# BenjSta/bernoulli-var-speech-codec

Measured on AMD Instinct MI355X. Metric: audio-seconds coded per wall-second (encode+decode), 22.05 kHz @ 3 kbit/s, higher is better.
Workload: dtype f32; 1 GPU; BASELINE configs[1]: batch 64 x 5 s utterances per GPU, config_varBitRate @ 3000 bit/s (35 bits/frame), full encode -> BigVGAN decode; one batch at a time on one stream; frames_per_utterance=430, weights=seeded synthetic (checkpoints are LFS pointers), gather=none, streams=1

## Files before the change

bernoulli-var-speech-codec_amd/csrc/bvc_internal.h:

```cpp
#pragma once
#include <hip/hip_runtime.h>
#include <stdint.h>
#include <string>
#include <vector>

#include "../../include/bvcodec.h"

namespace bvc {

void set_error(const char *fmt, ...);

#define BVC_HIP_TRY(expr)                                                              \
    do {                                                                               \
        hipError_t e_ = (expr);                                                        \
        if (e_ != hipSuccess) {                                                        \
            bvc::set_error("%s failed: %s (%s:%d)", #expr, hipGetErrorString(e_), __FILE__, __LINE__); \
            return BVC_EHIP;                                                           \
        }                                                                              \
    } while (0)

enum ProbeKind { PK_NONE = 0, PK_LINEAR = 1, PK_GRU = 2, PK_CONV = 3, PK_BATCHED = 4, PK_STFT = 5, PK_POST = 6 };
struct ProbeScope {
    hipStream_t s; int slot;
    ProbeScope(int kind, hipStream_t stream);
// ... 168 lines not shown
    const int   *mel_off;
    const float *mel_w;
    int num_mels;
    int kmax;
};
int launch_stft_logmel(const FrontendTables &t, const float *wav, int B, long long L, long long T,
                       int pad_left, float scale, float *mel, hipStream_t s, const long long *lens = nullptr);
__host__ __device__ inline long long ragged_frames(long long len, long long L, int pad_left) {
    len = len < 0 ? 0 : (len > L ? L : len);
    const long long pr = 1024 - 256 - pad_left;
    if (len <= pad_left || len <= pr) return 0;
    return (len + pad_left + pr - 1024) / 256 + 1;
}
int launch_ragged_bits(float *bits, const float *d_bits, float dflt, const long long *lens, int B, long long L, long long T,
                       int pad_left, hipStream_t s);
int launch_ragged_mask(float *codes, const long long *lens, int B, long long L, long long T, int z, int pad_left, hipStream_t s);

int launch_resample_poly(const float *x, int B, long long Lin, const double *h, int ntaps, int up, int down,
                         long long n_pre_remove, float *y, long long n_out, hipStream_t s);
int launch_peak_normalize(float *x, int B, long long L, hipStream_t s);
int launch_pack_codes(const float *codes, long long frames, int z, int nbits, unsigned char *out, hipStream_t s);
int launch_unpack_codes(const unsigned char *in, long long frames, int z, int nbits, float *codes, hipStream_t s);
int launch_pack_rows(const float *codes, const float *bits, int B, int k, int z, int kstride, unsigned char *out, hipStream_t s);
int launch_unpack_rows(const unsigned char *in, const unsigned char *present, const float *bits, const int *row_off, int B, int k,
                       int z, int kstride, float *codes, hipStream_t s);
int launch_conceal_select(const unsigned char *present, long long kstride, const float *bits, float dflt, const int *row_off, int B,
                          long long k, float *sel, hipStream_t s);

struct ConvLayer {
    int cin;
    int cout;
    int ntiles;
    int ks;
    int dil;
    const float *wp;
    const float *wp4;
    const float *wp2;
    const float *bias;
    const float *act_a;
    const float *act_ib;
    const float *aa_up;
    const float *aa_down;
};
enum ConvEpi { CE_STORE = 0, CE_RES = 1, CE_RES_ACC = 2, CE_RES_ACC_DIV = 3 };
#ifdef BVC_PHASE_PROBE
int phase_probe_read(unsigned long long *out, int reset);
#endif
struct ConvWindow {
    long long in_bs, out_bs, row_begin, t_origin;
    const int *row_age = nullptr;
    int age_rate = 0;
};
int conv_kernels_init();
enum : unsigned { AMPK_C8 = 1u, AMPK_C16 = 2u, AMPK_ALL = 3u };
unsigned amp_kernels_default();
struct AmpLaunch { long long tiles, workgroups; int tile_rows; };
extern AmpLaunch g_last_amp_launch;
int launch_snakebeta_test(const float *x, long long n, float a, float ib, float *y, hipStream_t s);
int launch_conv_mfma(const ConvLayer &c, const float *in, long long Lin, float *out, long long Lout,
                     int B, int epi, const float *res, const float *acc, float divisor, hipStream_t s,
                     const ConvWindow *win = nullptr, const long long *row_lim = nullptr,
                     long long in_bs = 0,
                     int shift = 0);
int launch_amp_pair(const ConvLayer &c1, const ConvLayer &c2, const float *x, long long L, float *out, int B, int epi,
                    const float *acc, float divisor, hipStream_t s, const ConvWindow *win = nullptr, unsigned kernels = AMPK_ALL,
                    bool sym = false,
                    long long bs = 0);
int launch_conv_post(const float *in, long long Lin, int C, int ks, const float *w, const float *bias,
                     const float *act_a, const float *act_ib, float div, float *wav, long long n_out,
                     int B, hipStream_t s, const ConvWindow *win = nullptr, const long long *n_rows = nullptr,
                     const float *aa_up = nullptr, const float *aa_down = nullptr,
                     bool sym = false,
                     long long in_bs = 0);
int launch_ragged_limits(long long *lim, const long long *frames, const long long *lengths, int B, long long T, long long n_max,
                         int n_up, const int *up_rates, hipStream_t s);

}
```

bernoulli-var-speech-codec_amd/csrc/k_vocoder.hip:

```cpp
#include <cstdlib>
#include <type_traits>

#include "bvc_internal.h"

namespace bvc {

typedef float f32x4 __attribute__((ext_vector_type(4)));

__device__ __forceinline__ void divide_if(bool div, f32x4 &v, float d) {
    if (div) {
        asm volatile("" ::: "memory");
#pragma unroll
        for (int e = 0; e < 4; ++e) v[e] = v[e] / d;
    }
}

__device__ __forceinline__ unsigned div_tpb(unsigned bid, unsigned tpb_magic) { return __umulhi(bid, tpb_magic); }
static inline unsigned tpb_magic_of(unsigned d) { return d <= 1u ? 0xFFFFFFFFu : (unsigned)(0x100000000ull / d) + 1u; }

__device__ __forceinline__ __amdgpu_buffer_rsrc_t rows_rsrc(const float *base, long long L, int C) {
    return __builtin_amdgcn_make_buffer_rsrc(const_cast<float *>(base), 0, (int)(L * C * 4), 0x00020000);
}
__device__ __forceinline__ f32x4 rows_load4(__amdgpu_buffer_rsrc_t rs, int row, int C, int c0) {
    return __builtin_bit_cast(f32x4, __builtin_amdgcn_raw_buffer_load_b128(rs, (row * C + c0) * 4, 0, 0));
// ... 190 lines not shown
    const int j0 = run * R, j1 = j0 + R < ndst ? j0 + R : ndst;
    if (j0 >= j1) return;
    const int last = L - 1 > 0x7FFFFFFFll ? 0x7FFFFFFF : (int)(L - 1);
    const int glo = src_first > 0 ? src_first : 0;
    const int ghi = src_first + nsrc - 1 < last ? src_first + nsrc - 1 : last;
    const f32x2 aa = *reinterpret_cast<const f32x2 *>(act_a + c), bb = *reinterpret_cast<const f32x2 *>(act_ib + c);
    float f[12], g[12];
#pragma unroll
    for (int k = 0; k < 12; ++k) { f[k] = fu[k]; g[k] = fd[k]; }
    auto pair = [&](int t, f32x2 &ev, f32x2 &od) {
        const int tc = t < 0 ? 0 : (t > last ? last : t);
        f32x2 xr[7];
#pragma unroll
        for (int k = 0; k < 7; ++k) {
            int q = tc - 3 + k;
            q = q < glo ? glo : (q > ghi ? ghi : q);
            xr[k] = *reinterpret_cast<const f32x2 *>(src + (q - src_first) * S + c);
        }
        f32x2 ue = splat2(f[1]) * xr[5], uo = splat2(f[0]) * xr[6];
#pragma unroll
        for (int k = 1; k < 6; ++k) {
            ue = __builtin_elementwise_fma(splat2(f[2 * k + 1]), xr[5 - k], ue);
            uo = __builtin_elementwise_fma(splat2(f[2 * k]), xr[6 - k], uo);
        }
        ev = snakebeta2(ue * splat2(2.0f), aa, bb);
        od = snakebeta2(uo * splat2(2.0f), aa, bb);
        if (t < 0) od = ev;
        if (t > last) ev = od;
    };
    f32x2 pe[6], po[6];
    const int tfirst = dst_first + j0;
#pragma unroll
    for (int k = 0; k < 6; ++k) pair(tfirst - 3 + k, pe[k], po[k]);
#pragma unroll 1
    for (int j = j0; j < j1; ++j) {
        const int t = dst_first + j;
        f32x2 ne, no;
        pair(t + 3, ne, no);
        f32x2 y = splat2(g[0]) * po[0];
#pragma unroll
        for (int k = 1; k < 6; ++k) {
            y = __builtin_elementwise_fma(splat2(g[2 * k - 1]), pe[k], y);
            y = __builtin_elementwise_fma(splat2(g[2 * k]), po[k], y);
        }
        y = __builtin_elementwise_fma(splat2(g[11]), ne, y);
        if (t < 0) y = splat2(0.0f);
        *reinterpret_cast<float2 *>(dst + j * S + c) = make_float2(y[0], y[1]);
#pragma unroll
        for (int k = 0; k < 5; ++k) { pe[k] = pe[k + 1]; po[k] = po[k + 1]; }
        pe[5] = ne; po[5] = no;
    }
}

template <int C, int MT, int OCC, bool ALIAS, int CS = 1, bool AA = false, bool SYM = false>
__global__ __launch_bounds__(256, OCC) void amp_pair_kernel(AmpArgs a) {
    static_assert(!(SYM && AA), "a filtered stage is a causal stage");
#ifdef BVC_PHASE_PROBE
    unsigned long long last_ = __builtin_readcyclecounter();
#endif
    extern __shared__ __attribute__((aligned(16))) float lds[];
    constexpr int S = C + 2;
    constexpr int NT = (C + 15) / 16;
    constexpr int C4 = C / 4;
    constexpr int TR = (4 / CS) * MT * 16;
    constexpr int NTL = NT / CS;
    static_assert((CS == 1 || CS == 2 || CS == 4) && NT % CS == 0, "the waves along the columns must divide the column tiles");
    constexpr int CGU = C4 < 16 / NTL ? C4 : 16 / NTL;
    constexpr bool W4 = C >= 32 && CGU % 4 == 0;
    const int tid = threadIdx.x, lane = tid & 63;
    const int wave = __builtin_amdgcn_readfirstlane(tid >> 6);
    const int r = lane & 15, g = lane >> 4;
    const int ks = a.ks, dil = a.dil;
    constexpr int AAH = AA ? 5 : 0;
    const int TT = TR - (ks - 1) - 2 * AAH;
    const unsigned nwg = gridDim.x, per = (nwg + 7u) >> 3;
    unsigned bid = (blockIdx.x & 7u) * per + (blockIdx.x >> 3);
    if (bid >= a.ntile) return;
    const int b = a.tiles_per_batch == 1 ? (int)bid : (int)div_tpb(bid, a.tpb_magic);
    const long long t0 = a.row_begin + (long long)(bid - (unsigned)b * (unsigned)a.tiles_per_batch) * TT;
    const int halo1 = (ks - 1) * dil;
    const int rows1 = TR + halo1;
    float *t1 = lds;
    float *t2 = (ALIAS || AA) ? lds : lds + rows1 * S;
    const float *xb = a.x + (long long)b * a.bs;
    const long long tbase = t0 - (SYM ? (ks - 1) / 2 : ks - 1) - AAH;
    const int rowsA = rows1 > TR + ks - 1 ? rows1 : TR + ks - 1;
    float *traw = lds + rowsA * S;
    (void)traw;

    if constexpr (AA) {
        constexpr int NLD = ((TR + 10 * 5 + 2 * AAH) * C4 + 255) / 256;
        f32x4 v[NLD];
        const int total = (rows1 + 2 * AAH) * C4;
        const __amdgpu_buffer_rsrc_t rs = rows_rsrc(xb, a.L, C);
        const int xfirst = (int)(tbase - halo1) - AAH;
#pragma unroll
        for (int i = 0; i < NLD; ++i) {
            const int idx = tid + i * 256;
            const int row = idx / C4, c4 = idx - row * C4;
            v[i] = rows_load4(rs, xfirst + row, C, c4 * 4);
        }
#pragma unroll
        for (int i = 0; i < NLD; ++i) {
            const int idx = tid + i * 256;
            if (idx < total) {
                const int row = idx / C4, c4 = idx - row * C4;
                float2 *dst = reinterpret_cast<float2 *>(traw + row * S + c4 * 4);
                dst[0] = make_float2(v[i][0], v[i][1]);
                dst[1] = make_float2(v[i][2], v[i][3]);
            }
        }
        __syncthreads();
        aa_rows<C>(traw, xfirst, rows1 + 2 * AAH, a.L, t1, xfirst + AAH, rows1, S, a.a1, a.ib1, a.fu1, a.fd1);
    } else {
        constexpr int NLD = ((TR + 10 * 5) * C4 + 255) / 256;
        f32x4 v[NLD];
        const int total = rows1 * C4;
        const __amdgpu_buffer_rsrc_t rs = rows_rsrc(xb, a.L, C);
        const int tfirst = (int)(tbase - (SYM ? halo1 / 2 : halo1));
#pragma unroll
        for (int i = 0; i < NLD; ++i) {
            const int idx = tid + i * 256;
            const int row = idx / C4, c4 = idx - row * C4;
            v[i] = rows_load4(rs, tfirst + row, C, c4 * 4);
        }
#pragma unroll
        for (int i = 0; i < NLD; ++i) {
            const int idx = tid + i * 256;
            if (idx < total) {
                const int row = idx / C4, c4 = idx - row * C4;
                const f32x4 aa = *reinterpret_cast<const f32x4 *>(a.a1 + c4 * 4);
                const f32x4 bb = *reinterpret_cast<const f32x4 *>(a.ib1 + c4 * 4);
                f32x4 o;
#pragma unroll
                for (int e = 0; e < 4; e += 2) {
                    const f32x2 o2 = snakebeta2((f32x2){v[i][e], v[i][e + 1]}, (f32x2){aa[e], aa[e + 1]}, (f32x2){bb[e], bb[e + 1]});
                    o[e] = o2[0]; o[e + 1] = o2[1];
                }
                float2 *dst = reinterpret_cast<float2 *>(t1 + row * S + c4 * 4);
                dst[0] = make_float2(o[0], o[1]);
                dst[1] = make_float2(o[2], o[3]);
            }
        }
    }
    __syncthreads();
    PHASE(0);

    const int mbase = (wave / CS) * MT * 16;
    const int nt0 = (wave % CS) * NTL;
    f32x4 acc[MT][NTL];
    auto mma = [&](const float *tile, int d, const float *wp) {
#pragma unroll
        for (int i = 0; i < MT; ++i)
#pragma unroll
            for (int n = 0; n < NTL; ++n) acc[i][n] = (f32x4){0.f, 0.f, 0.f, 0.f};
        const float *wl = wp + lane;
        constexpr int CPT = C4 / CGU;
        const int nch = ks * CPT;
        constexpr int G4 = W4 ? CGU / 4 : CGU;
        typedef typename std::conditional<W4, f32x4, float>::type BW;
        BW bcur[G4][NTL], bnxt[G4][NTL];
        auto loadb = [&](BW (&dstb)[G4][NTL], int q) {
            if constexpr (W4) {
                const f32x4 *wq = reinterpret_cast<const f32x4 *>(wp) + (long long)q * G4 * NT * 64 + lane;
#pragma unroll
                for (int u = 0; u < G4; ++u)
#pragma unroll
                    for (int n = 0; n < NTL; ++n) dstb[u][n] = wq[(u * NT + nt0 + n) * 64];
            } else {
                const float *wq = wl + (long long)q * CGU * NT * 64;
#pragma unroll
                for (int u = 0; u < CGU; ++u)
#pragma unroll
                    for (int n = 0; n < NTL; ++n) dstb[u][n] = wq[(u * NT + nt0 + n) * 64];
            }
        };
        auto bfrag = [&](const BW (&bw)[G4][NTL], int u, int n) -> float {
            if constexpr (W4) return bw[u >> 2][n][u & 3];
            else return bw[u][n];
        };
        auto compute = [&](const BW (&bw)[G4][NTL], int q) {
            const int j = q / CPT, cg0 = (q - j * CPT) * CGU;
            const float *arow = tile + (mbase + r + j * d) * S + g;
#pragma unroll
            for (int u = 0; u < CGU; ++u) {
                float av[MT];
#pragma unroll
                for (int i = 0; i < MT; ++i) av[i] = arow[i * 16 * S + (cg0 + u) * 4];
#pragma unroll
                for (int i = 0; i < MT; ++i)
#pragma unroll
                    for (int n = 0; n < NTL; ++n)
                        acc[i][n] = __builtin_amdgcn_mfma_f32_16x16x4f32(av[i], bfrag(bw, u, n), acc[i][n], 0, 0, 0);
            }
        };
        loadb(bcur, 0);
        if constexpr (BVC_AMP_PINGPONG && C == 32) {
            int q = 0;
#pragma unroll 1
            for (; q + 1 < nch; q += 2) {
                loadb(bnxt, q + 1);
                __builtin_amdgcn_sched_barrier(0);
                compute(bcur, q);
                __builtin_amdgcn_sched_barrier(0);
                loadb(bcur, q + 2 < nch ? q + 2 : nch - 1);
                __builtin_amdgcn_sched_barrier(0);
                compute(bnxt, q + 1);
                __builtin_amdgcn_sched_barrier(0);
            }
            if (q < nch) compute(bcur, q);
        } else {
#pragma unroll 1
            for (int q = 0; q < nch; ++q) {
                loadb(bnxt, q + 1 < nch ? q + 1 : nch - 1);
                __builtin_amdgcn_sched_barrier(0);
                compute(bcur, q);
                __builtin_amdgcn_sched_barrier(0);
#pragma unroll
                for (int u = 0; u < G4; ++u)
#pragma unroll
                    for (int n = 0; n < NTL; ++n) bcur[u][n] = bnxt[u][n];
            }
        }
    };

    auto mma_small = [&](const float *tile, int d, const float *wp, auto ks_c) {
        constexpr int KS = decltype(ks_c)::value;
        static_assert(NT == 1 || KS == 0, "mma_small is for one 16-column tile");
        float wreg[KS][C4];
        const float *wl = wp + lane;
#pragma unroll
        for (int j = 0; j < KS; ++j)
#pragma unroll
            for (int c = 0; c < C4; ++c) wreg[j][c] = wl[(j * C4 + c) * NT * 64];
#pragma unroll
        for (int i = 0; i < MT; ++i) acc[i][0] = (f32x4){0.f, 0.f, 0.f, 0.f};
#pragma unroll
        for (int j = 0; j < KS; ++j) {
            const float *arow = tile + (mbase + r + j * d) * S + g;
#pragma unroll
            for (int c = 0; c < C4; ++c) {
                float av[MT];
#pragma unroll
                for (int i = 0; i < MT; ++i) av[i] = arow[i * 16 * S + c * 4];
#pragma unroll
                for (int i = 0; i < MT; ++i)
                    acc[i][0] = __builtin_amdgcn_mfma_f32_16x16x4f32(av[i], wreg[j][c], acc[i][0], 0, 0, 0);
            }
        }
    };
    auto conv = [&](const float *tile, int d, const float *wp) {
        if constexpr (C <= 16) {
            if (ks == 11) { mma_small(tile, d, wp, std::integral_constant<int, 11>()); return; }
            if (ks == 7) { mma_small(tile, d, wp, std::integral_constant<int, 7>()); return; }
            if (ks == 3) { mma_small(tile, d, wp, std::integral_constant<int, 3>()); return; }
        }
        mma(tile, d, wp);
    };

    conv(t1, dil, a.w1);
    PHASE(1);
    if (ALIAS || AA) __syncthreads();
    const long long zr64 = -(tbase + amp_t_origin(a, b));
    const int zrow = zr64 <= 0 ? 0 : (zr64 > TR ? TR : (int)zr64);
    const long long ze64 = a.L - tbase;
    const int zend = !SYM ? TR : (ze64 <= 0 ? 0 : (ze64 > TR ? TR : (int)ze64));
    if constexpr (AA) {
#pragma unroll
        for (int n = 0; n < NTL; ++n) {
            const int col = (nt0 + n) * 16 + r;
            if (col < C) {
                const float bias = a.b1[col];
#pragma unroll
                for (int i = 0; i < MT; ++i)
#pragma unroll
                    for (int e = 0; e < 4; ++e) traw[(mbase + i * 16 + g * 4 + e) * S + col] = acc[i][n][e] + bias;
            }
        }
        for (int idx = tid; idx < (ks - 1 + 2 * AAH) * S; idx += 256) t2[(TR - 2 * AAH) * S + idx] = 0.0f;
        __syncthreads();
        aa_rows<C>(traw, (int)tbase, TR, a.L, t2, (int)tbase + AAH, TR - 2 * AAH, S, a.a2, a.ib2, a.fu2, a.fd2);
    } else {
    for (int idx = tid; idx < (ks - 1) * S; idx += 256) t2[TR * S + idx] = 0.0f;
    if constexpr (C == 8) {
        const int col = r & 7, e0 = (r >> 3) * 2;
        const float bias = a.b1[col], aa = a.a2[col], bb = a.ib2[col];
#pragma unroll
        for (int i = 0; i < MT; ++i) {
            const float a0 = acc[i][0][0], a1 = acc[i][0][1], a2 = acc[i][0][2], a3 = acc[i][0][3];
            const float hi0 = __int_as_float(__builtin_amdgcn_update_dpp(0, __float_as_int(a2), 0x118, 0xf, 0xf, false));
            const float hi1 = __int_as_float(__builtin_amdgcn_update_dpp(0, __float_as_int(a3), 0x118, 0xf, 0xf, false));
            const float v0 = r < 8 ? a0 : hi0, v1 = r < 8 ? a1 : hi1;
            const int row = mbase + i * 16 + g * 4 + e0;
            const f32x2 s2 = snakebeta2((f32x2){v0 + bias, v1 + bias}, splat2(aa), splat2(bb));
            t2[row * S + col] = (row >= zrow && (!SYM || row < zend)) ? s2[0] : 0.0f;
            t2[(row + 1) * S + col] = (row + 1 >= zrow && (!SYM || row + 1 < zend)) ? s2[1] : 0.0f;
        }
    } else {
        auto s2_tile = [&](auto edge_c) {
            constexpr bool EDGE = decltype(edge_c)::value;
#pragma unroll
            for (int n = 0; n < NTL; ++n) {
                const int col = (nt0 + n) * 16 + r;
                if (col < C) {
                    const float bias = a.b1[col], aa = a.a2[col], bb = a.ib2[col];
#pragma unroll
                    for (int i = 0; i < MT; ++i)
#pragma unroll
                        for (int e = 0; e < 4; e += 2) {
                            const int row = mbase + i * 16 + g * 4 + e;
                            const f32x2 u2 = (f32x2){acc[i][n][e] + bias, acc[i][n][e + 1] + bias};
                            const f32x2 s2 = snakebeta2(u2, splat2(aa), splat2(bb));
                            t2[row * S + col] = (!EDGE || (row >= zrow && (!SYM || row < zend))) ? s2[0] : 0.0f;
                            t2[(row + 1) * S + col] = (!EDGE || (row + 1 >= zrow && (!SYM || row + 1 < zend))) ? s2[1] : 0.0f;
                        }
                }
            }
        };
        if (zrow > 0 || (SYM && zend < TR)) s2_tile(std::true_type());
        else                                s2_tile(std::false_type());
    }
    }
    (void)zrow; (void)zend;
    __syncthreads();
    PHASE(2);

    const long long ob = (long long)b * a.bs + t0 * C;
    constexpr int NLD3 = (TR * C4 + 255) / 256;
    const long long rows_left = a.L - t0;
    const int nvalid4 = (int)(rows_left < TT ? rows_left : TT) * C4;
    f32x4 resq[NLD3], accq[NLD3];
    const bool with_acc = a.epi >= CE_RES_ACC;
#pragma unroll
    for (int i = 0; i < NLD3; ++i) {
        const int idx = tid + i * 256;
        const int idc = idx < nvalid4 ? idx : 0;
        resq[i] = reinterpret_cast<const f32x4 *>(a.x + ob)[idc];
        accq[i] = with_acc ? reinterpret_cast<const f32x4 *>(a.acc + ob)[idc] : (f32x4){0.f, 0.f, 0.f, 0.f};
    }
    PHASE(3);
    conv(t2, 1, a.w2);
    PHASE(4);
    if (ALIAS || AA) __syncthreads();
#pragma unroll
    for (int n = 0; n < NTL; ++n) {
        const int col = (nt0 + n) * 16 + r;
        if (col >= C) continue;
        const float bias = a.b2[col];
#pragma unroll
        for (int i = 0; i < MT; ++i)
#pragma unroll
            for (int e = 0; e < 4; ++e) t1[(mbase + i * 16 + g * 4 + e) * S + col] = acc[i][n][e] + bias;
    }
    __syncthreads();
#pragma unroll
    for (int i = 0; i < NLD3; ++i) {
        const int idx = tid + i * 256;
        if (idx >= nvalid4) continue;
        const int row = idx / C4, c4 = idx - row * C4;
        const float2 lo = *reinterpret_cast<const float2 *>(t1 + row * S + c4 * 4);
        const float2 hi = *reinterpret_cast<const float2 *>(t1 + row * S + c4 * 4 + 2);
        f32x4 v = (f32x4){lo.x, lo.y, hi.x, hi.y};
#pragma unroll
        for (int e = 0; e < 4; ++e) {
            float o = v[e] + resq[i][e];
            if (a.epi >= CE_RES_ACC) o = accq[i][e] + o;
            v[e] = o;
        }
        divide_if(a.epi == CE_RES_ACC_DIV, v, a.divisor);
        reinterpret_cast<f32x4 *>(a.out + ob)[idx] = v;
    }
    PHASE(5);
}

unsigned amp_kernels_default() {
    return (getenv("BVC_NO_AMP8") == nullptr ? AMPK_C8 : 0u) | (getenv("BVC_NO_AMP16") == nullptr ? AMPK_C16 : 0u);
}

template <int D>
__device__ __forceinline__ int pair_row(int m) { return (m / D) * (2 * D) + m % D; }
template <int D>
__device__ __forceinline__ int row_pos(int rho, int H) {
    const int blk = rho / (2 * D), w = rho - blk * (2 * D);
    return w >= D ? H + blk * D + (w - D) : blk * D + w;
}
template <int KS, int D, int MT2>
struct Amp8Geom {
    static constexpr int NP = 4 * MT2 * 16;
    static constexpr int NPE = (NP / D) * D;
    static constexpr int TR1 = 2 * NPE;
    static constexpr int TR = 2 * NP;
    static constexpr int TT = TR1 - (KS - 1);
    static constexpr int HALO1 = (KS - 1) * D;
    static constexpr int ROWS1 = TR1 + HALO1;
    static constexpr int H1 = NP + ((KS + 1) / 2) * D;
    static constexpr int H2 = NP + (KS + 1) / 2;
    static constexpr int S = 10;
    static constexpr int LDS_ROWS = 2 * H1 > TR ? 2 * H1 : TR;
    static constexpr size_t LDS_BYTES = (size_t)LDS_ROWS * S * sizeof(float);
};

template <int KS, int D, int MT2, int OCC>
__global__ __launch_bounds__(256, OCC) void amp_pair8_kernel(AmpArgs a) {
    extern __shared__ __attribute__((aligned(16))) float lds[];
    using G = Amp8Geom<KS, D, MT2>;
    constexpr int C = 8, S = G::S, NP = G::NP, NPE = G::NPE, TR = G::TR, TT = G::TT, H1 = G::H1, H2 = G::H2;
    constexpr int NLD = (G::ROWS1 * 2 + 255) / 256;
    const int tid = threadIdx.x, lane = tid & 63;
    const int wave = __builtin_amdgcn_readfirstlane(tid >> 6);
    const int r = lane & 15, g = lane >> 4;
    const unsigned per = (a.ntile + 7u) >> 3, nli = gridDim.x >> 3;
    const unsigned xcd = blockIdx.x & 7u;
    unsigned li = blockIdx.x >> 3;
    const unsigned run_end = (xcd + 1u) * per < a.ntile ? (xcd + 1u) * per : a.ntile;
    if (xcd * per + li >= run_end) return;

    float w1reg[KS + 1][2], w2reg[KS + 1][2];
#pragma unroll
    for (int k = 0; k <= KS; ++k)
#pragma unroll
        for (int q = 0; q < 2; ++q) {
            w1reg[k][q] = a.w1[(k * 2 + q) * 64 + lane];
            w2reg[k][q] = a.w2[(k * 2 + q) * 64 + lane];
        }
    const f32x4 aa1 = *reinterpret_cast<const f32x4 *>(a.a1 + (tid & 1) * 4);
    const f32x4 bb1 = *reinterpret_cast<const f32x4 *>(a.ib1 + (tid & 1) * 4);
    const int p = g >> 1, co0 = (g & 1) * 4;
    const f32x4 bias1 = *reinterpret_cast<const f32x4 *>(a.b1 + co0), aa2 = *reinterpret_cast<const f32x4 *>(a.a2 + co0);
    const f32x4 bb2 = *reinterpret_cast<const f32x4 *>(a.ib2 + co0), bias2 = *reinterpret_cast<const f32x4 *>(a.b2 + co0);
// ... 355 lines not shown
        int per_cu = 0, dev = 0, cus = 0;
        if (hipGetDevice(&dev) != hipSuccess || hipDeviceGetAttribute(&cus, hipDeviceAttributeMultiprocessorCount, dev) != hipSuccess ||
            hipOccupancyMaxActiveBlocksPerMultiprocessor(&per_cu, reinterpret_cast<const void *>(amp_pair16_kernel<KS, D, MT, OCC>), 256,
                                                         Amp16Geom<KS, D, MT>::LDS_BYTES) != hipSuccess) {
            set_error("amp_pair16: occupancy query failed");
            return -1;
        }
        slots = (per_cu > 0 ? per_cu : 1) * cus;
    }
    return slots;
}
template <int KS, int D, int MT, int OCC>
static int launch_amp16_t(AmpArgs a, int B, hipStream_t s) {
    using G = Amp16Geom<KS, D, MT>;
    a.tiles_per_batch = (int)((a.L - a.row_begin + G::TT - 1) / G::TT);
    if (a.tiles_per_batch <= 0) return BVC_OK;
    a.tpb_magic = tpb_magic_of((unsigned)a.tiles_per_batch);
    if ((unsigned long long)a.tiles_per_batch * a.tiles_per_batch * (unsigned long long)B >= 0x100000000ull) { set_error("vocoder: tile count beyond the reciprocal's range"); return BVC_EINVAL; }
    const int slots = amp16_slots<KS, D, MT, OCC>();
    if (slots <= 0) return BVC_EHIP;
    ProbeScope probe(PK_CONV, s);
    const unsigned ntile = (unsigned)(a.tiles_per_batch * (long long)B);
    a.ntile = ntile;
    const unsigned grid = ntile < (unsigned)slots ? ((ntile + 7u) & ~7u) : ((unsigned)slots & ~7u);
    g_last_amp_launch = {(long long)ntile, (long long)grid, G::TT};
    hipLaunchKernelGGL((amp_pair16_kernel<KS, D, MT, OCC>), dim3(grid), dim3(256), G::LDS_BYTES, s, a);
    BVC_HIP_TRY(hipGetLastError());
    return BVC_OK;
}
template <int KS, int MT> struct Amp16Occ { static constexpr int V = MT >= 4 ? 2 : (KS == 3 ? 4 : KS == 7 ? 3 : 2); };
template <int MT>
static int launch_amp16(AmpArgs a, int B, hipStream_t s) {
    switch (a.ks * 8 + a.dil) {
        case 3 * 8 + 1:  return launch_amp16_t<3, 1, MT, Amp16Occ<3, MT>::V>(a, B, s);
        case 3 * 8 + 3:  return launch_amp16_t<3, 3, MT, Amp16Occ<3, MT>::V>(a, B, s);
        case 3 * 8 + 5:  return launch_amp16_t<3, 5, MT, Amp16Occ<3, MT>::V>(a, B, s);
        case 7 * 8 + 1:  return launch_amp16_t<7, 1, MT, Amp16Occ<7, MT>::V>(a, B, s);
        case 7 * 8 + 3:  return launch_amp16_t<7, 3, MT, Amp16Occ<7, MT>::V>(a, B, s);
        case 7 * 8 + 5:  return launch_amp16_t<7, 5, MT, Amp16Occ<7, MT>::V>(a, B, s);
        case 11 * 8 + 1: return launch_amp16_t<11, 1, (MT > 4 ? 4 : MT), Amp16Occ<11, MT>::V>(a, B, s);
        case 11 * 8 + 3: return launch_amp16_t<11, 3, (MT > 4 ? 4 : MT), Amp16Occ<11, MT>::V>(a, B, s);
        case 11 * 8 + 5: return launch_amp16_t<11, 5, (MT > 4 ? 4 : MT), Amp16Occ<11, MT>::V>(a, B, s);
        default: return -1;
    }
}
template <int MT>
static bool amp16_slots_all() {
    return amp16_slots<3, 1, MT, Amp16Occ<3, MT>::V>() > 0 && amp16_slots<3, 3, MT, Amp16Occ<3, MT>::V>() > 0 && amp16_slots<3, 5, MT, Amp16Occ<3, MT>::V>() > 0 &&
           amp16_slots<7, 1, MT, Amp16Occ<7, MT>::V>() > 0 && amp16_slots<7, 3, MT, Amp16Occ<7, MT>::V>() > 0 && amp16_slots<7, 5, MT, Amp16Occ<7, MT>::V>() > 0 &&
           amp16_slots<11, 1, (MT > 4 ? 4 : MT), Amp16Occ<11, MT>::V>() > 0 && amp16_slots<11, 3, (MT > 4 ? 4 : MT), Amp16Occ<11, MT>::V>() > 0 &&
           amp16_slots<11, 5, (MT > 4 ? 4 : MT), Amp16Occ<11, MT>::V>() > 0;
}

template <int C, int MT, int OCC, bool ALIAS, int CS = 1, bool AA = false, bool SYM = false>
static int launch_amp_t(AmpArgs a, int B, hipStream_t s) {
    constexpr int TR = (4 / CS) * MT * 16;
    const int TT = TR - (a.ks - 1) - (AA ? 10 : 0);
    a.tiles_per_batch = (int)((a.L - a.row_begin + TT - 1) / TT);
    if (a.tiles_per_batch <= 0) return BVC_OK;
    a.tpb_magic = tpb_magic_of((unsigned)a.tiles_per_batch);
    if ((unsigned long long)a.tiles_per_batch * a.tiles_per_batch * (unsigned long long)B >= 0x100000000ull) { set_error("vocoder: tile count beyond the reciprocal's range"); return BVC_EINVAL; }
    const int rows1 = TR + (a.ks - 1) * a.dil;
    const size_t lds = AA ? (size_t)((rows1 > TR + a.ks - 1 ? rows1 : TR + a.ks - 1) + rows1 + 10) * (C + 2) * sizeof(float)
                          : (size_t)(rows1 + (ALIAS ? 0 : TR + (a.ks - 1))) * (C + 2) * sizeof(float);
    if (AA && a.L + TR > 0x7FFFFFFFll) { set_error("amp_pair: %lld rows are beyond the anti-aliased kernel's row index", a.L); return BVC_EINVAL; }
    if (lds > 160 * 1024 || TT <= 0) { set_error("amp_pair tile needs %zu B of LDS", lds); return BVC_EINVAL; }
    ProbeScope probe(PK_CONV, s);
    const unsigned ntile = (unsigned)(a.tiles_per_batch * (long long)B);
    a.ntile = ntile;
    {
        static bool attr = false;
        if (!attr) { BVC_HIP_TRY(hipFuncSetAttribute(reinterpret_cast<const void *>(amp_pair_kernel<C, MT, OCC, ALIAS, CS, AA, SYM>), hipFuncAttributeMaxDynamicSharedMemorySize, 160 * 1024)); attr = true; }
    }
    g_last_amp_launch = {(long long)ntile, (long long)((ntile + 7u) & ~7u), TT};
    hipLaunchKernelGGL((amp_pair_kernel<C, MT, OCC, ALIAS, CS, AA, SYM>), dim3((ntile + 7u) & ~7u), dim3(256), lds, s, a);
    BVC_HIP_TRY(hipGetLastError());
    return BVC_OK;
}

TilePlan g_last_amp_cut = {0, 0, 0, 0};
static constexpr int AMP64_FIXED_ROWS = 1;
TilePlan amp_pair_cut(long long L, int B, int ks, int force_height, bool legacy) {
    static const int heights[4] = {128, 112, 96, 80}, slots[4] = {512, 512, 512, 512};
    if (!force_height && !legacy) return tile_plan(L, B, heights, slots, 4, AMP64_FIXED_ROWS, ks - 1);
    int one = force_height ? 0 : heights[0];
    for (int h : heights) if (h == force_height) one = h;
    if (!one) return {0, 0, 0, 0};
    return tile_plan(L, B, &one, slots, 1, AMP64_FIXED_ROWS, ks - 1);
}

int launch_amp_pair(const ConvLayer &c1, const ConvLayer &c2, const float *x, long long L, float *out, int B, int epi,
                    const float *acc, float divisor, hipStream_t s, const ConvWindow *win, unsigned kernels, bool sym, long long bs) {
    if (B <= 0 || L <= 0) return BVC_OK;
    if (c1.cin != c1.cout || c2.cin != c1.cin || c2.ks != c1.ks || c2.dil != 1 || !c1.act_a || !c2.act_a) {
        set_error("amp_pair: unsupported layer pair");
        return BVC_EINVAL;
    }
    AmpArgs a;
    a.x = x; a.out = out; a.acc = acc; a.L = L;
    a.w1 = c1.wp; a.b1 = c1.bias; a.a1 = c1.act_a; a.ib1 = c1.act_ib;
    a.w2 = c2.wp; a.b2 = c2.bias; a.a2 = c2.act_a; a.ib2 = c2.act_ib;
    if (c1.cin >= 32) {
        if (!c1.wp4 || !c2.wp4) { set_error("amp_pair: layer pair without the 16-byte weight packing"); return BVC_EINVAL; }
        a.w1 = c1.wp4; a.w2 = c2.wp4;
    }
    a.divisor = divisor; a.epi = epi; a.ks = c1.ks; a.dil = c1.dil; a.tiles_per_batch = 0;
    a.bs = win ? win->in_bs : (bs ? bs : L * c1.cin);
    a.row_begin = win ? win->row_begin : 0;
    a.t_origin = win ? win->t_origin : 0;
    a.row_age = win ? win->row_age : nullptr;
    a.age_rate = win ? win->age_rate : 0;
    a.fu1 = c1.aa_up; a.fd1 = c1.aa_down; a.fu2 = c2.aa_up; a.fd2 = c2.aa_down;
    const bool wide = c1.cin >= 128;
    if (wide) {
        if (c1.cin != 128 && c1.cin != 256) { set_error("amp_pair: unsupported channel count %d", c1.cin); return BVC_EINVAL; }
        if (c1.aa_up || c2.aa_up || c1.aa_down || c2.aa_down) { set_error("amp_pair: anti-aliased activations are not implemented on a stage of %d channels (64 at most)", c1.cin); return BVC_EINVAL; }
        if (sym) { set_error("amp_pair: symmetric layers are not implemented on a stage of %d channels (64 at most)", c1.cin); return BVC_EINVAL; }
        if (L + 512 > 0x7FFFFFFFll / c1.cin / 4) { set_error("amp_pair: %lld rows of %d channels are beyond the kernel's row index", L, c1.cin); return BVC_EINVAL; }
    }
    if (c1.aa_up || c2.aa_up) {
        if (!c1.aa_up || !c1.aa_down || !c2.aa_up || !c2.aa_down) { set_error("amp_pair: a pair is filtered on both activations or on none"); return BVC_EINVAL; }
        if (win) { set_error("amp_pair: an anti-aliased pair looks ahead and has no streaming window"); return BVC_EINVAL; }
        switch (c1.cin) {
            case 64: return launch_amp_t<64, 6, 2, true, 4, true>(a, B, s);
            case 32: return launch_amp_t<32, 2, 3, true, 1, true>(a, B, s);
            case 16: return launch_amp_t<16, 2, 4, true, 1, true>(a, B, s);
            case 8:  return launch_amp_t<8, 4, 4, true, 1, true>(a, B, s);
            default: set_error("amp_pair: unsupported channel count %d", c1.cin); return BVC_EINVAL;
// ... 11 lines not shown
            case 8:  return launch_amp_t<8, 4, 4, true, 1, false, true>(a, B, s);
            default: set_error("amp_pair: unsupported channel count %d", c1.cin); return BVC_EINVAL;
        }
    }
    if (bs) { set_error("amp_pair: a batch stride of its own belongs to a symmetric stage's view"); return BVC_EINVAL; }
    const long long new_rows = L - a.row_begin;
    if (wide) {
        const bool short_win = win && new_rows <= 32 - (c1.ks - 1);
        if (c1.cin == 256) {
            if (short_win) return launch_amp_t<256, 2, 1, true, 4>(a, B, s);
            const char *force = win ? nullptr : getenv("BVC_AMP256_TR");
            const int tr = force ? atoi(force) : 64;
            if (tr == 64) return launch_amp_t<256, 4, 1, true, 4>(a, B, s);
            if (tr == 96) return launch_amp_t<256, 6, 1, true, 4>(a, B, s);
            set_error("amp_pair: BVC_AMP256_TR=%s is not a compiled tile height", force); return BVC_EINVAL;
        }
        if (short_win) return launch_amp_t<128, 2, 2, true, 4>(a, B, s);
        const char *force = win ? nullptr : getenv("BVC_AMP128_TR");
        const int tr = force ? atoi(force) : 64;
        if (tr == 64) return launch_amp_t<128, 4, 2, true, 4>(a, B, s);
        if (tr == 128) return launch_amp_t<128, 8, 1, true, 4>(a, B, s);
        set_error("amp_pair: BVC_AMP128_TR=%s is not a compiled tile height", force); return BVC_EINVAL;
    }
    if (win && c1.cin == 64 && new_rows <= 32 - (c1.ks - 1)) return launch_amp_t<64, 2, 2, true, 4>(a, B, s);
    if (win && c1.cin == 64 && new_rows <= 2 * (64 - (c1.ks - 1))) return launch_amp_t<64, 1, 2, true>(a, B, s);
    static const int s32 = getenv("BVC_AMP32S") ? atoi(getenv("BVC_AMP32S")) : 3;
    if (win && c1.cin == 32 && new_rows <= s32 * (64 - (c1.ks - 1))) return launch_amp_t<32, 1, 3, true>(a, B, s);
    if (c1.cin == 8 && c1.wp2 && c2.wp2 && (kernels & AMPK_C8)) {
        AmpArgs a8 = a;
        a8.w1 = c1.wp2; a8.w2 = c2.wp2;
        const int rc8 = (win && new_rows <= 128) ? launch_amp8<1, 4>(a8, B, s) : launch_amp8<2, 2>(a8, B, s);
        if (rc8 != -1) return rc8;
    }
    switch (c1.cin) {
        case 64: {
            static const bool rows = getenv("BVC_AMP64") && atoi(getenv("BVC_AMP64")) == 0;
            if (rows) return launch_amp_t<64, 2, 2, true>(a, B, s);
            int tr = 128;
            if (!win) {
                const char *force = getenv("BVC_AMP64_TR");
                const TilePlan cut = amp_pair_cut(new_rows, B, c1.ks, force ? atoi(force) : 0, tile_cut_legacy());
                if (cut.height == 0) { set_error("amp_pair: BVC_AMP64_TR=%s is not a compiled tile height", force ? force : ""); return BVC_EINVAL; }
                g_last_amp_cut = cut;
                tile_trace("amp_pair64", new_rows, (long long)B * 100 + c1.ks, cut.height, 0, cut.tiles, 512, cut.rounds);
                tr = cut.height;
            }
            switch (tr) {
                case 80:  return launch_amp_t<64, 5, 2, true, 4>(a, B, s);
                case 96:  return launch_amp_t<64, 6, 2, true, 4>(a, B, s);
                case 112: return launch_amp_t<64, 7, 2, true, 4>(a, B, s);
                default:  return launch_amp_t<64, 8, 2, true, 4>(a, B, s);
            }
        }
        case 32: return launch_amp_t<32, 4, 3, true>(a, B, s);
        case 16: {
            if ((kernels & AMPK_C16) && !win) {
                const int rc16 = launch_amp16<4>(a, B, s);
                if (rc16 != -1) return rc16;
            }
            return launch_amp_t<16, 2, 4, false>(a, B, s);
        }
        case 8:  return launch_amp_t<8, 4, 4, true>(a, B, s);
        default: set_error("amp_pair: unsupported channel count %d", c1.cin); return BVC_EINVAL;
    }
}

template <int CIN, int NTW, int MT, bool NSPLIT = false, int SHIFT = 0>
static int launch_one(const ConvArgs &a, int B, hipStream_t s) {
    constexpr int TT = (NSPLIT ? 1 : 4) * MT * 16;
    ConvArgs k = a;
    k.tiles_per_batch = (int)((a.Lout - a.row_begin + TT - 1) / TT);
    if (k.tiles_per_batch <= 0) return BVC_OK;
    const size_t lds = (size_t)(TT + (a.ks - 1) * a.dil) * (CIN + 2) * sizeof(float);
    if (lds > 160 * 1024) { set_error("conv tile needs %zu B of LDS", lds); return BVC_EINVAL; }
    constexpr int NPW = NTW * (NSPLIT ? 4 : 1);
    dim3 grid((unsigned)(k.tiles_per_batch * (long long)B), (unsigned)((a.ntiles + NPW - 1) / NPW));
    auto kern = conv_mfma_kernel<CIN, NTW, MT, NSPLIT, SHIFT>;
    ProbeScope probe(PK_CONV, s);
    hipLaunchKernelGGL(kern, grid, dim3(256), lds, s, k);
    BVC_HIP_TRY(hipGetLastError());
    return BVC_OK;
}

template <int CIN, int NTW, int MT, bool NSPLIT = false, int SHIFT = 0>
static int allow_big_lds() {
    BVC_HIP_TRY(hipFuncSetAttribute(reinterpret_cast<const void *>(conv_mfma_kernel<CIN, NTW, MT, NSPLIT, SHIFT>),
                                    hipFuncAttributeMaxDynamicSharedMemorySize, 160 * 1024));
    return BVC_OK;
}

__global__ void snakebeta_test_kernel(const float *__restrict__ x, long long n, float a, float ib, float *__restrict__ y) {
    for (long long i = ((long long)blockIdx.x * blockDim.x + threadIdx.x) * 2; i < n; i += (long long)gridDim.x * blockDim.x * 2) {
        if (i + 1 < n && !(i & 2)) {
            const f32x2 v = snakebeta2((f32x2){x[i], x[i + 1]}, splat2(a), splat2(ib));
            y[i] = v[0];
            y[i + 1] = v[1];
        } else {
            y[i] = snakebeta(x[i], a, ib);
            if (i + 1 < n) y[i + 1] = snakebeta(x[i + 1], a, ib);
        }
    }
}

int launch_snakebeta_test(const float *x, long long n, float a, float ib, float *y, hipStream_t s) {
    if (n <= 0) return BVC_OK;
    hipLaunchKernelGGL(snakebeta_test_kernel, dim3(256), dim3(256), 0, s, x, n, a, ib, y);
    BVC_HIP_TRY(hipGetLastError());
// ... 202 lines not shown
```

bernoulli-var-speech-codec_amd/csrc/model.hip:

```cpp
#include <cmath>
#include <cstdio>
#include <map>
#include <memory>

#include "bvc_host.h"

using namespace bvc;

namespace {

typedef std::map<std::string, const bvc_tensor *> TensorMap;

template <typename T>
int upload_raw(bvc_model *m, const T *h, int64_t n, const T **dev) {
    void *d = nullptr;
    const size_t bytes = (size_t)n * sizeof(T);
    BVC_HIP_TRY(hipMalloc(&d, bytes ? bytes : 16));
    m->allocs.push_back(d);
    if (bytes) BVC_HIP_TRY(hipMemcpy(d, h, bytes, hipMemcpyHostToDevice));
    *dev = static_cast<const T *>(d);
    return BVC_OK;
}
template <typename T>
int upload(bvc_model *m, const std::vector<T> &host, const T **dev) { return upload_raw(m, host.data(), (int64_t)host.size(), dev); }
// ... 551 lines not shown
        set_error("no HIP device visible: the gfx950 kernels cannot run (there is no CPU fallback)");
        return BVC_ENODEVICE;
    }
    TensorMap tm;
    for (int i = 0; i < n_tensors; ++i)
        if (tensors[i].name) tm[tensors[i].name] = &tensors[i];
    std::unique_ptr<bvc_model> m(new bvc_model());
    m->cfg = *cfg;
    if ((rc = conv_kernels_init())) return rc;
    if ((rc = skinny_kernels_init())) return rc;
    {
        const char *ng = getenv("BVC_NO_GRAPH");
        m->use_graph = !(ng && ng[0] == '1');
        const char *sb = getenv("BVC_SIDE_BRANCH");
        m->side_branch = (sb && sb[0] == '1');
        const char *mw = getenv("BVC_MTW");
        if (mw && (mw[0] == '2' || mw[0] == '4')) m->mtw = mw[0] - '0';
        const char *ua = getenv("BVC_UNFUSED_AMP");
        m->fused_amp = !(ua && ua[0] == '1');
        m->amp_kernels = amp_kernels_default();
        const char *np = getenv("BVC_NO_PRECOMP");
        m->precomp_pz = !(np && np[0] == '1') && !m->side_branch;
    }
    if ((rc = build_frontend(m.get(), tm))) return rc;
    if ((rc = build_bvrnn(m.get(), tm))) return rc;
    {
        const char *rr = getenv("BVC_RECURRENCE");
        m->recurrence = (rr && strcmp(rr, "layers") == 0) ? RS_LAYERS : (rr && strcmp(rr, "persistent") == 0) ? RS_PERSISTENT : RS_AUTO;
    }
    if ((rc = build_flow(m.get()))) return rc;
    if ((rc = build_vocoder(m.get(), tm))) return rc;
    BVC_HIP_TRY(hipDeviceSynchronize());
    *out = m.release();
    return BVC_OK;
}

void bvc_model_destroy(bvc_model *m) { delete m; }

int bvc_model_set_option(bvc_model *m, const char *name, int32_t value) {
    if (!m || !name) { set_error("bvc_model_set_option: null argument"); return BVC_EINVAL; }
    if (strcmp(name, "recurrence") == 0) {
        if (value < 0 || value > 2) { set_error("bvc_model_set_option: recurrence must be 0 (persistent), 1 (layers) or 2 (auto)"); return BVC_EINVAL; }
        m->recurrence = value;
        return BVC_OK;
    }
    if (strcmp(name, "flow_spin_limit") == 0) {
        if (value < 1) { set_error("bvc_model_set_option: flow_spin_limit must be positive"); return BVC_EINVAL; }
        m->flow_spin_limit = (unsigned)value;
        return BVC_OK;
    }
    for (const auto &f : {std::make_pair("flow_debug_withhold", &m->flow_debug_withhold), std::make_pair("flow_debug_nofill", &m->flow_debug_nofill),
                          std::make_pair("decode_fold", &m->decode_fold), std::make_pair("encode_fold", &m->encode_fold)})
        if (strcmp(name, f.first) == 0) { *f.second = value != 0; return BVC_OK; }
    for (const auto &k : {std::make_pair("vocoder_c16_kernel", AMPK_C16), std::make_pair("vocoder_full_tiles", AMPK_C8)})
        if (strcmp(name, k.first) == 0) { m->amp_kernels = value ? (m->amp_kernels | k.second) : (m->amp_kernels & ~k.second); return BVC_OK; }
    set_error("bvc_model_set_option: unknown option '%s'", name);
    return BVC_EINVAL;
}

int bvc_model_get_option(const bvc_model *m, const char *name, int32_t *value) {
    if (!m || !name || !value) { set_error("bvc_model_get_option: null argument"); return BVC_EINVAL; }
    if (strcmp(name, "recurrence") == 0) { *value = m->recurrence; return BVC_OK; }
    if (strcmp(name, "decode_fold") == 0) { *value = m->decode_fold; return BVC_OK; }
    if (strcmp(name, "encode_fold") == 0) { *value = m->encode_fold; return BVC_OK; }
    if (strcmp(name, "flow_resident") == 0) { *value = m->flow_resident ? 1 : 0; return BVC_OK; }
    if (strcmp(name, "flow_supported") == 0) { *value = m->flow_perh > 0 ? 1 : 0; return BVC_OK; }
    if (strcmp(name, "compute_units") == 0) { *value = m->cu_count; return BVC_OK; }
    set_error("bvc_model_get_option: unknown option '%s'", name);
    return BVC_EINVAL;
}

int bvc_model_status(const bvc_model *m, uint32_t *code) {
    if (!m) { set_error("null model"); return BVC_EINVAL; }
    if (m->h_status) BVC_HIP_TRY(hipDeviceSynchronize());
    const unsigned v = take_status(m);
    if (code) *code = v;
    if (v) {
        set_error("a persistent recurrence kernel gave up waiting (frame %u, layer %u): its results are invalid",
                  (v & 0x7FFFFFFFu) >> 4, (v & 15u));
        return BVC_ETIMEOUT;
    }
    return BVC_OK;
}

int bvc_model_poll_status(const bvc_model *m, uint32_t *code) {
    if (!m) { set_error("null model"); return BVC_EINVAL; }
    const unsigned v = take_status(m);
    if (code) *code = v;
    if (v) {
        set_error("a persistent recurrence kernel gave up waiting (frame %u, layer %u): the results of the call that has just been "
                  "synchronised are invalid.  All its workgroups must be resident together - is another process using this GPU?",
                  (v & 0x7FFFFFFFu) >> 4, (v & 15u));
        return BVC_ETIMEOUT;
    }
    return BVC_OK;
}

}
```

Before: 7094 audio-seconds/s.

## Add software-pipelined MFMA loop variant for C=32 vocoder AMP pair kernel

Adds an LP template variant of the amp_pair kernel for the offline C=32 shape. In the MMA inner loop it double-buffers the A-operand LDS reads so the next fragment loads overlap the current MFMAs, with sched_barriers fixing the order. It also loads the input tile with a strided row-per-thread scheme and keeps per-column bias and activation parameters in registers. The variant is on by default for windowless C=32 launches and can be turned off with an env var or model option. The cost is higher register pressure at occupancy 3, which could cause spills.

After: 7096 audio-seconds/s, median of 2. About the same (+0.0%).

```diff
diff --git a/bernoulli-var-speech-codec_amd/csrc/bvc_internal.h b/bernoulli-var-speech-codec_amd/csrc/bvc_internal.h
--- a/bernoulli-var-speech-codec_amd/csrc/bvc_internal.h
+++ b/bernoulli-var-speech-codec_amd/csrc/bvc_internal.h
@@ -244,7 +244,7 @@
     int age_rate = 0;
 };
 int conv_kernels_init();
-enum : unsigned { AMPK_C8 = 1u, AMPK_C16 = 2u, AMPK_ALL = 3u };
+enum : unsigned { AMPK_C8 = 1u, AMPK_C16 = 2u, AMPK_LOOP = 4u, AMPK_ALL = 7u };
 unsigned amp_kernels_default();
 struct AmpLaunch { long long tiles, workgroups; int tile_rows; };
 extern AmpLaunch g_last_amp_launch;
diff --git a/bernoulli-var-speech-codec_amd/csrc/k_vocoder.hip b/bernoulli-var-speech-codec_amd/csrc/k_vocoder.hip
--- a/bernoulli-var-speech-codec_amd/csrc/k_vocoder.hip
+++ b/bernoulli-var-speech-codec_amd/csrc/k_vocoder.hip
@@ -266,9 +266,10 @@
     }
 }
 
-template <int C, int MT, int OCC, bool ALIAS, int CS = 1, bool AA = false, bool SYM = false>
+template <int C, int MT, int OCC, bool ALIAS, int CS = 1, bool AA = false, bool SYM = false, bool LP = false>
 __global__ __launch_bounds__(256, OCC) void amp_pair_kernel(AmpArgs a) {
     static_assert(!(SYM && AA), "a filtered stage is a causal stage");
+    static_assert(!LP || (!AA && !SYM && C >= 32 && 256 % (C / 4) == 0), "the ordered loop is the offline C = 32 shape's");
 #ifdef BVC_PHASE_PROBE
     unsigned long long last_ = __builtin_readcyclecounter();
 #endif
@@ -301,6 +302,17 @@
     const int rowsA = rows1 > TR + ks - 1 ? rows1 : TR + ks - 1;
     float *traw = lds + rowsA * S;
     (void)traw;
+    const int mbase = (wave / CS) * MT * 16;
+    const int nt0 = (wave % CS) * NTL;
+    float cb1[NTL], ca2[NTL], cib2[NTL], cb2[NTL];
+    if constexpr (LP) {
+#pragma unroll
+        for (int n = 0; n < NTL; ++n) {
+            const int col = (nt0 + n) * 16 + r;
+            cb1[n] = a.b1[col]; ca2[n] = a.a2[col]; cib2[n] = a.ib2[col]; cb2[n] = a.b2[col];
+        }
+    }
+    (void)cb1; (void)ca2; (void)cib2; (void)cb2;
 
     if constexpr (AA) {
         constexpr int NLD = ((TR + 10 * 5 + 2 * AAH) * C4 + 255) / 256;
@@ -326,6 +338,37 @@
         }
         __syncthreads();
         aa_rows<C>(traw, xfirst, rows1 + 2 * AAH, a.L, t1, xfirst + AAH, rows1, S, a.a1, a.ib1, a.fu1, a.fd1);
+    } else if constexpr (LP) {
+        constexpr int NLD = ((TR + 10 * 5) * C4 + 255) / 256;
+        constexpr int RPG = 256 / C4;
+        f32x4 v[NLD];
+        const int total = rows1 * C4;
+        const __amdgpu_buffer_rsrc_t rs = rows_rsrc(xb, a.L, C);
+        const int row0 = tid / C4, c4 = tid - row0 * C4;
+        const int tfirst = (int)(tbase - halo1) + row0;
+        const f32x4 aa = *reinterpret_cast<const f32x4 *>(a.a1 + c4 * 4);
+        const f32x4 bb = *reinterpret_cast<const f32x4 *>(a.ib1 + c4 * 4);
+#pragma unroll
+        for (int i = 0; i < NLD; ++i) v[i] = rows_load4(rs, tfirst + i * RPG, C, c4 * 4);
+#pragma unroll
+        for (int i = 0; i < NLD; ++i) asm volatile("" : "+v"(v[i]));
+        float *dst0 = t1 + row0 * S + c4 * 4;
+#pragma unroll
+        for (int i = 0; i < NLD; ++i) {
+            if (i * 256 < total) {
+                f32x4 o;
+#pragma unroll
+                for (int e = 0; e < 4; e += 2) {
+                    const f32x2 o2 = snakebeta2((f32x2){v[i][e], v[i][e + 1]}, (f32x2){aa[e], aa[e + 1]}, (f32x2){bb[e], bb[e + 1]});
+                    o[e] = o2[0]; o[e + 1] = o2[1];
+                }
+                if (tid + i * 256 < total) {
+                    float2 *dst = reinterpret_cast<float2 *>(dst0 + i * RPG * S);
+                    dst[0] = make_float2(o[0], o[1]);
+                    dst[1] = make_float2(o[2], o[3]);
+                }
+            }
+        }
     } else {
         constexpr int NLD = ((TR + 10 * 5) * C4 + 255) / 256;
         f32x4 v[NLD];
@@ -360,10 +403,8 @@
     __syncthreads();
     PHASE(0);
 
-    const int mbase = (wave / CS) * MT * 16;
-    const int nt0 = (wave % CS) * NTL;
     f32x4 acc[MT][NTL];
-    auto mma = [&](const float *tile, int d, const float *wp) {
+    auto mma = [&](const float *tile, int d, const float *wp) __attribute__((always_inline)) {
 #pragma unroll
         for (int i = 0; i < MT; ++i)
 #pragma unroll
@@ -408,7 +449,75 @@
                         acc[i][n] = __builtin_amdgcn_mfma_f32_16x16x4f32(av[i], bfrag(bw, u, n), acc[i][n], 0, 0, 0);
             }
         };
+        constexpr int GR = 1;
+        constexpr int NP = CGU / GR;
+        static_assert(!LP || (NP % 2 == 0), "the two operand sets take turns and a chunk ends on the first");
+        float pa0[MT][GR], pa1[MT][GR];
+        (void)pa0; (void)pa1;
+        auto aptr = [&](int q) __attribute__((always_inline)) -> const float * {
+            const int j = q / CPT, cg0 = (q - j * CPT) * CGU;
+            return tile + (mbase + r + j * d) * S + g + cg0 * 4;
+        };
+        auto lda = [&](float (&dst)[GR], const float *ap, int i, int p) __attribute__((always_inline)) {
+#pragma unroll
+            for (int e = 0; e < GR; ++e) dst[e] = ap[i * 16 * S + (p * GR + e) * 4];
+        };
+        auto set_step = [&](const BW (&bw)[G4][NTL], int p, const float (&cur)[MT][GR], float (&nxt)[MT][GR], const float *an, int pn) __attribute__((always_inline)) {
+#pragma unroll
+            for (int e = 0; e < GR; ++e) {
+#pragma unroll
+                for (int i = 0; i < MT; ++i) {
+#pragma unroll
+                    for (int n = 0; n < NTL; ++n)
+                        acc[i][n] = __builtin_amdgcn_mfma_f32_16x16x4f32(cur[i][e], bfrag(bw, p * GR + e, n), acc[i][n], 0, 0, 0);
+                    if (e == 0) {
+                        lda(nxt[i], an, i, pn);
+                        __builtin_amdgcn_sched_barrier(0);
+                    }
+                }
+            }
+            __builtin_amdgcn_sched_barrier(0);
+        };
+        auto compute_lp = [&](const BW (&bw)[G4][NTL], int q, int qn) __attribute__((always_inline)) {
+            const float *ap = aptr(q), *an = aptr(qn);
+#pragma unroll
+            for (int p = 0; p < NP; p += 2) {
+                set_step(bw, p, pa0, pa1, ap, p + 1);
+                set_step(bw, p + 1, pa1, pa0, p + 2 < NP ? ap : an, p + 2 < NP ? p + 2 : 0);
+            }
+        };
         loadb(bcur, 0);
+        if constexpr (LP) {
+#pragma unroll
+            for (int i = 0; i < MT; ++i) lda(pa0[i], aptr(0), i, 0);
+            __builtin_amdgcn_sched_barrier(0);
+            if constexpr (BVC_AMP_PINGPONG && C == 32) {
+                int q = 0;
+#pragma unroll 1
+                for (; q + 1 < nch; q += 2) {
+                    loadb(bnxt, q + 1);
+                    __builtin_amdgcn_sched_barrier(0);
+                    compute_lp(bcur, q, q + 1);
+                    loadb(bcur, q + 2 < nch ? q + 2 : nch - 1);
+                    __builtin_amdgcn_sched_barrier(0);
+                    compute_lp(bnxt, q + 1, q + 2 < nch ? q + 2 : nch - 1);
+                }
+                if (q < nch) compute_lp(bcur, q, q);
+            } else {
+#pragma unroll 1
+                for (int q = 0; q < nch; ++q) {
+                    const int qn = q + 1 < nch ? q + 1 : nch - 1;
+                    loadb(bnxt, qn);
+                    __builtin_amdgcn_sched_barrier(0);
+                    compute_lp(bcur, q, qn);
+#pragma unroll
+                    for (int u = 0; u < G4; ++u)
+#pragma unroll
+                        for (int n = 0; n < NTL; ++n) bcur[u][n] = bnxt[u][n];
+                }
+            }
+            return;
+        }
         if constexpr (BVC_AMP_PINGPONG && C == 32) {
             int q = 0;
 #pragma unroll 1
@@ -463,7 +572,7 @@
             }
         }
     };
-    auto conv = [&](const float *tile, int d, const float *wp) {
+    auto conv = [&](const float *tile, int d, const float *wp) __attribute__((always_inline)) {
         if constexpr (C <= 16) {
             if (ks == 11) { mma_small(tile, d, wp, std::integral_constant<int, 11>()); return; }
             if (ks == 7) { mma_small(tile, d, wp, std::integral_constant<int, 7>()); return; }
@@ -517,7 +626,7 @@
             for (int n = 0; n < NTL; ++n) {
                 const int col = (nt0 + n) * 16 + r;
                 if (col < C) {
-                    const float bias = a.b1[col], aa = a.a2[col], bb = a.ib2[col];
+                    const float bias = LP ? cb1[n] : a.b1[col], aa = LP ? ca2[n] : a.a2[col], bb = LP ? cib2[n] : a.ib2[col];
 #pragma unroll
                     for (int i = 0; i < MT; ++i)
 #pragma unroll
@@ -560,7 +669,7 @@
     for (int n = 0; n < NTL; ++n) {
         const int col = (nt0 + n) * 16 + r;
         if (col >= C) continue;
-        const float bias = a.b2[col];
+        const float bias = LP ? cb2[n] : a.b2[col];
 #pragma unroll
         for (int i = 0; i < MT; ++i)
 #pragma unroll
@@ -588,7 +697,8 @@
 }
 
 unsigned amp_kernels_default() {
-    return (getenv("BVC_NO_AMP8") == nullptr ? AMPK_C8 : 0u) | (getenv("BVC_NO_AMP16") == nullptr ? AMPK_C16 : 0u);
+    const char *lp = getenv("BVC_AMP_LOOP");
+    return (getenv("BVC_NO_AMP8") == nullptr ? AMPK_C8 : 0u) | (getenv("BVC_NO_AMP16") == nullptr ? AMPK_C16 : 0u) | (lp && atoi(lp) == 0 ? 0u : AMPK_LOOP);
 }
 
 template <int D>
@@ -1050,7 +1160,7 @@
            amp16_slots<11, 5, (MT > 4 ? 4 : MT), Amp16Occ<11, MT>::V>() > 0;
 }
 
-template <int C, int MT, int OCC, bool ALIAS, int CS = 1, bool AA = false, bool SYM = false>
+template <int C, int MT, int OCC, bool ALIAS, int CS = 1, bool AA = false, bool SYM = false, bool LP = false>
 static int launch_amp_t(AmpArgs a, int B, hipStream_t s) {
     constexpr int TR = (4 / CS) * MT * 16;
     const int TT = TR - (a.ks - 1) - (AA ? 10 : 0);
@@ -1068,10 +1178,10 @@
     a.ntile = ntile;
     {
         static bool attr = false;
-        if (!attr) { BVC_HIP_TRY(hipFuncSetAttribute(reinterpret_cast<const void *>(amp_pair_kernel<C, MT, OCC, ALIAS, CS, AA, SYM>), hipFuncAttributeMaxDynamicSharedMemorySize, 160 * 1024)); attr = true; }
+        if (!attr) { BVC_HIP_TRY(hipFuncSetAttribute(reinterpret_cast<const void *>(amp_pair_kernel<C, MT, OCC, ALIAS, CS, AA, SYM, LP>), hipFuncAttributeMaxDynamicSharedMemorySize, 160 * 1024)); attr = true; }
     }
     g_last_amp_launch = {(long long)ntile, (long long)((ntile + 7u) & ~7u), TT};
-    hipLaunchKernelGGL((amp_pair_kernel<C, MT, OCC, ALIAS, CS, AA, SYM>), dim3((ntile + 7u) & ~7u), dim3(256), lds, s, a);
+    hipLaunchKernelGGL((amp_pair_kernel<C, MT, OCC, ALIAS, CS, AA, SYM, LP>), dim3((ntile + 7u) & ~7u), dim3(256), lds, s, a);
     BVC_HIP_TRY(hipGetLastError());
     return BVC_OK;
 }
@@ -1189,7 +1299,8 @@
                 default:  return launch_amp_t<64, 8, 2, true, 4>(a, B, s);
             }
         }
-        case 32: return launch_amp_t<32, 4, 3, true>(a, B, s);
+        case 32: if (!win && (kernels & AMPK_LOOP)) return launch_amp_t<32, 4, 3, true, 1, false, false, true>(a, B, s);
+                 return launch_amp_t<32, 4, 3, true>(a, B, s);
         case 16: {
             if ((kernels & AMPK_C16) && !win) {
                 const int rc16 = launch_amp16<4>(a, B, s);
diff --git a/bernoulli-var-speech-codec_amd/csrc/model.hip b/bernoulli-var-speech-codec_amd/csrc/model.hip
--- a/bernoulli-var-speech-codec_amd/csrc/model.hip
+++ b/bernoulli-var-speech-codec_amd/csrc/model.hip
@@ -627,7 +627,7 @@
     for (const auto &f : {std::make_pair("flow_debug_withhold", &m->flow_debug_withhold), std::make_pair("flow_debug_nofill", &m->flow_debug_nofill),
                           std::make_pair("decode_fold", &m->decode_fold), std::make_pair("encode_fold", &m->encode_fold)})
         if (strcmp(name, f.first) == 0) { *f.second = value != 0; return BVC_OK; }
-    for (const auto &k : {std::make_pair("vocoder_c16_kernel", AMPK_C16), std::make_pair("vocoder_full_tiles", AMPK_C8)})
+    for (const auto &k : {std::make_pair("vocoder_c16_kernel", AMPK_C16), std::make_pair("vocoder_full_tiles", AMPK_C8), std::make_pair("vocoder_amp_loop", AMPK_LOOP)})
         if (strcmp(name, k.first) == 0) { m->amp_kernels = value ? (m->amp_kernels | k.second) : (m->amp_kernels & ~k.second); return BVC_OK; }
     set_error("bvc_model_set_option: unknown option '%s'", name);
     return BVC_EINVAL;
```
